# jipolanco/PencilArrays.jl

Hardware: NVIDIA B200
Metric: transpose_GiB_per_s (higher is better)
Workload: dtype c128 (bytes; pure data movement)

## Files before the change

include/pa_b200.h:

```cpp
#ifndef PA_B200_H
#define PA_B200_H

#include <stddef.h>
#include <stdint.h>

#ifdef __cplusplus
extern "C" {
#endif

#define PA_MAX_DIMS 8
#define PA_MAX_TOPO 7
#define PA_UNIQUE_ID_BYTES 128

typedef enum pa_status {
  PA_OK = 0,
  PA_EINVAL = 1,
  PA_EINCOMPAT = 2,
  PA_EDIM = 3,
  PA_ECUDA = 4,
  PA_ENCCL = 5,
  PA_ENOMEM = 6,
  PA_ESTATE = 7,
  PA_ENOGPU = 8
} pa_status;
// ... 79 lines not shown
  int64_t recv_count;
  int64_t remote_recv_offset;
} pa_peer_info;
pa_status pa_plan_get_peer(const pa_plan* plan, int n , pa_peer_info* info);

typedef struct pa_block_desc {
  int nd;
  int64_t extent[PA_MAX_DIMS];
  int64_t src_stride[PA_MAX_DIMS];
  int64_t dst_stride[PA_MAX_DIMS];
  int64_t src_offset;
  int64_t dst_offset;
  int kernel_class;
  int vec_bytes;
} pa_block_desc;
pa_status pa_plan_get_block(const pa_plan* plan, int op, int n ,
                            pa_block_desc* desc);
pa_status pa_plan_get_chunk(const pa_plan* plan, int op, int n, int part, int nparts,
                            pa_block_desc* desc, int64_t* wire_offset, int64_t* wire_bytes);

pa_status pa_pack(pa_plan* plan, int n, const void* src, void* buf, void* stream);
pa_status pa_unpack(pa_plan* plan, int n, const void* recv_buf, void* dst, void* stream);
pa_status pa_copy_self(pa_plan* plan, const void* src, void* dst, void* stream);
pa_status pa_put(pa_plan* plan, int n, const void* src, void* peer_dst, void* stream);
pa_status pa_get(pa_plan* plan, int n, const void* peer_src, void* dst, void* stream);
pa_status pa_put_all(pa_plan* plan, const void* src, void* const* peers, int max_ctas,
                     void* stream);
pa_status pa_get_all(pa_plan* plan, void* const* peers, void* dst, int max_ctas, void* stream);
pa_status pa_permute_local(pa_plan* plan, const void* src, void* dst,
                           void* scratch, void* stream);
pa_status pa_box_copy(int nd, const int64_t* extent, const int64_t* src_stride,
                      const int64_t* dst_stride, int elsize, const void* src,
                      void* dst, void* stream, pa_block_desc* chosen );

pa_status pa_comm_unique_id(void* id128);
pa_status pa_comm_init_rank(const void* id128, int nranks, int rank, pa_comm** out);
pa_status pa_comm_init_local(int nranks, int rank, pa_comm** out);
void pa_comm_destroy(pa_comm* c);
pa_status pa_comm_flags_export(pa_comm* c, void* handle64, int64_t* offset);
pa_status pa_comm_flags_import(pa_comm* c, int rank, const void* handle64, int64_t offset);

#define PA_IPC_HANDLE_BYTES 64
pa_status pa_ipc_export(const void* devptr, void* handle64, int64_t* offset);
pa_status pa_ipc_import(const void* handle64, int64_t offset, void** mapped);
pa_status pa_ipc_release(const void* handle64);
pa_status pa_plan_set_window(pa_plan* plan, const void* local_dst, int n, void* peer_dst);
pa_status pa_plan_set_recv_window(pa_plan* plan, int n, void* peer_recv_buf);

pa_status pa_transpose(pa_plan* plan, pa_comm* comm, const void* src, void* dst,
                       unsigned flags, void* stream);
pa_status pa_wait(pa_plan* plan, void* stream);
pa_status pa_transpose_host(pa_plan* plan, pa_comm* comm, const void* host_src,
                            void* host_dst, unsigned flags);

pa_status pa_host_chain_create(int n, pa_plan* const* plans, pa_comm* comm,
                               pa_host_chain** out);
void pa_host_chain_destroy(pa_host_chain* c);
pa_status pa_host_chain_submit(pa_host_chain* c, const void* host_src, void* host_dst,
                               int64_t* ticket );
pa_status pa_host_chain_wait(pa_host_chain* c, int64_t ticket);
pa_status pa_host_chain_buffer(pa_host_chain* c, int slot, int which, void** devptr,
                               int64_t* bytes);
pa_status pa_host_chain_time_begin(pa_host_chain* c);
pa_status pa_host_chain_time_end(pa_host_chain* c, float* ms);

pa_status pa_io_sizes(const pa_pencil* p, int n_extra, const int64_t* extra_dims, int elsize,
// ... 23 lines not shown
```

pencilarrays.jl_b200/_lib.py:

```python
from __future__ import annotations

import ctypes as C
import os

PA_MAX_DIMS = 8
PA_MAX_TOPO = 7
PA_UNIQUE_ID_BYTES = 128

PA_OK, PA_EINVAL, PA_EINCOMPAT, PA_EDIM, PA_ECUDA, PA_ENCCL, PA_ENOMEM, PA_ESTATE, PA_ENOGPU = range(9)

PA_POINT_TO_POINT = 0
PA_ALLTOALLV = 1
PA_PEER_PUT = 2
PA_PEER_GET = 3
PA_IPC_HANDLE_BYTES = 64

PA_WAITALL = 1
PA_NO_OVERLAP = 2
PA_STAGE_SELF = 4
PA_FFT_FORWARD = 8
PA_FFT_BACKWARD = 16

_HERE = os.path.dirname(os.path.abspath(__file__))
LIB_PATH = os.path.join(_HERE, "libpa_b200.so")


class PlanInfo(C.Structure):
    _fields_ = [
        ("dim", C.c_int), ("nproc", C.c_int), ("self_index", C.c_int), ("same_perm", C.c_int),
        ("elsize", C.c_int), ("method", C.c_int),
        ("length_in", C.c_int64), ("length_out", C.c_int64), ("length_self", C.c_int64),
        ("send_bytes", C.c_int64), ("recv_bytes", C.c_int64),
    ]


class PeerInfo(C.Structure):
    _fields_ = [
        ("world_rank", C.c_int), ("is_self", C.c_int),
        ("send_offset", C.c_int64), ("send_count", C.c_int64),
        ("recv_offset", C.c_int64), ("recv_count", C.c_int64),
        ("remote_recv_offset", C.c_int64),
    ]


class BlockDesc(C.Structure):
    _fields_ = [
        ("nd", C.c_int),
        ("extent", C.c_int64 * PA_MAX_DIMS),
        ("src_stride", C.c_int64 * PA_MAX_DIMS),
        ("dst_stride", C.c_int64 * PA_MAX_DIMS),
        ("src_offset", C.c_int64), ("dst_offset", C.c_int64),
        ("kernel_class", C.c_int), ("vec_bytes", C.c_int),
    ]


class Timings(C.Structure):
    _fields_ = [("total_ms", C.c_float), ("pack_ms", C.c_float),
                ("exchange_ms", C.c_float), ("unpack_ms", C.c_float)]


_P = C.c_void_p
_I64P = C.POINTER(C.c_int64)
_IP = C.POINTER(C.c_int)
SIGNATURES = {
    "pa_version": (C.c_char_p, []),
    "pa_strerror": (C.c_char_p, [C.c_int]),
    "pa_last_error": (C.c_char_p, []),
    "pa_launch_count": (C.c_int64, []),
    "pa_device_count": (C.c_int, []),
    "pa_set_device": (C.c_int, [C.c_int]),
    "pa_set_tunable": (C.c_int, [C.c_char_p, C.c_int64]),
    "pa_dims_create": (C.c_int, [C.c_int, C.c_int, _I64P]),
    "pa_topology_create": (C.c_int, [C.c_int, _I64P, C.c_int, C.POINTER(_P)]),
    "pa_topology_destroy": (None, [_P]),
    "pa_topology_info": (C.c_int, [_P, _IP, _I64P, _IP, _IP, _I64P]),
    "pa_topology_rank_of": (C.c_int, [_P, _I64P, _IP]),
    "pa_topology_line": (C.c_int, [_P, C.c_int, _IP]),
    "pa_pencil_create": (C.c_int, [_P, C.c_int, _I64P, _IP, _IP, _P, C.POINTER(_P)]),
    "pa_pencil_destroy": (None, [_P]),
    "pa_pencil_range": (C.c_int, [_P, _I64P, C.c_int, _I64P, _I64P]),
    "pa_pencil_size_local": (C.c_int, [_P, C.c_int, _I64P]),
    "pa_pencil_buffers": (C.c_int, [_P, C.POINTER(_P), _I64P, C.POINTER(_P), _I64P]),
    "pa_pencil_reserve": (C.c_int, [_P, C.c_int64, C.c_int64]),
    "pa_plan_create": (C.c_int, [_P, _P, C.c_int, _I64P, C.c_int, C.c_int, C.POINTER(_P)]),
    "pa_plan_destroy": (None, [_P]),
    "pa_plan_get_info": (C.c_int, [_P, C.POINTER(PlanInfo)]),
    "pa_plan_get_peer": (C.c_int, [_P, C.c_int, C.POINTER(PeerInfo)]),
    "pa_plan_get_block": (C.c_int, [_P, C.c_int, C.c_int, C.POINTER(BlockDesc)]),
    "pa_plan_get_chunk": (C.c_int, [_P, C.c_int, C.c_int, C.c_int, C.c_int, C.POINTER(BlockDesc),
                                    _I64P, _I64P]),
    "pa_pack": (C.c_int, [_P, C.c_int, _P, _P, _P]),
    "pa_unpack": (C.c_int, [_P, C.c_int, _P, _P, _P]),
    "pa_put": (C.c_int, [_P, C.c_int, _P, _P, _P]),
    "pa_get": (C.c_int, [_P, C.c_int, _P, _P, _P]),
    "pa_put_all": (C.c_int, [_P, _P, C.POINTER(_P), C.c_int, _P]),
    "pa_get_all": (C.c_int, [_P, C.POINTER(_P), _P, C.c_int, _P]),
    "pa_copy_self": (C.c_int, [_P, _P, _P, _P]),
    "pa_permute_local": (C.c_int, [_P, _P, _P, _P, _P]),
    "pa_box_copy": (C.c_int, [C.c_int, _I64P, _I64P, _I64P, C.c_int, _P, _P, _P,
                              C.POINTER(BlockDesc)]),
    "pa_comm_unique_id": (C.c_int, [_P]),
    "pa_comm_init_rank": (C.c_int, [_P, C.c_int, C.c_int, C.POINTER(_P)]),
    "pa_comm_init_local": (C.c_int, [C.c_int, C.c_int, C.POINTER(_P)]),
    "pa_comm_destroy": (None, [_P]),
    "pa_comm_flags_export": (C.c_int, [_P, _P, _I64P]),
    "pa_comm_flags_import": (C.c_int, [_P, C.c_int, _P, C.c_int64]),
    "pa_ipc_export": (C.c_int, [_P, _P, _I64P]),
    "pa_ipc_import": (C.c_int, [_P, C.c_int64, C.POINTER(_P)]),
    "pa_ipc_release": (C.c_int, [_P]),
    "pa_plan_set_window": (C.c_int, [_P, _P, C.c_int, _P]),
    "pa_plan_set_recv_window": (C.c_int, [_P, C.c_int, _P]),
    "pa_transpose": (C.c_int, [_P, _P, _P, _P, C.c_uint, _P]),
    "pa_wait": (C.c_int, [_P, _P]),
    "pa_transpose_host": (C.c_int, [_P, _P, _P, _P, C.c_uint]),
    "pa_host_chain_create": (C.c_int, [C.c_int, C.POINTER(_P), _P, C.POINTER(_P)]),
    "pa_host_chain_destroy": (None, [_P]),
    "pa_host_chain_submit": (C.c_int, [_P, _P, _P, _I64P]),
    "pa_host_chain_wait": (C.c_int, [_P, C.c_int64]),
    "pa_host_chain_time_begin": (C.c_int, [_P]),
    "pa_host_chain_time_end": (C.c_int, [_P, C.POINTER(C.c_float)]),
    "pa_host_chain_buffer": (C.c_int, [_P, C.c_int, C.c_int, C.POINTER(_P), _I64P]),
    "pa_io_sizes": (C.c_int, [_P, C.c_int, _I64P, C.c_int, C.c_int, _I64P, _I64P, _I64P, _I64P, _I64P]),
    "pa_io_run_offset": (C.c_int, [_P, C.c_int, _I64P, C.c_int, C.c_int, C.c_int64, _I64P]),
    "pa_io_write": (C.c_int, [_P, C.c_int, _I64P, C.c_int, C.c_int, _P, C.c_char_p, C.c_int64]),
    "pa_io_read": (C.c_int, [_P, C.c_int, _I64P, C.c_int, C.c_int, _P, C.c_char_p, C.c_int64]),
    "pa_plan_timings": (C.c_int, [_P, C.POINTER(Timings)]),
    "pa_plan_enable_timing": (C.c_int, [_P, C.c_int]),
}


def _load():
    if not os.path.exists(LIB_PATH):
        raise ImportError(
# ... 54 lines not shown
```

pencilarrays.jl_b200/csrc/capi.cpp:

```cpp
#include <algorithm>
#include <new>
#include <vector>

#include "pa_internal.hpp"

using namespace pa;

#define GUARD(expr)                    \
  try {                                \
    expr                               \
  } catch (const std::bad_alloc&) {    \
    set_error("out of host memory");   \
    return PA_ENOMEM;                  \
  } catch (...) {                      \
    set_error("unexpected exception"); \
    return PA_EINVAL;                  \
  }

extern "C" {

const char* pa_version(void) { return "pa_b200 0.2.0 (sm_100a)"; }

const char* pa_strerror(pa_status s) {
  switch (s) {
    case PA_OK: return "success";
    case PA_EINVAL: return "invalid argument";
    case PA_EINCOMPAT: return "pencil configurations are not compatible for transposition";
    case PA_EDIM: return "array dimensions do not match the pencil";
    case PA_ECUDA: return "CUDA error";
    case PA_ENCCL: return "NCCL error";
    case PA_ENOMEM: return "out of memory";
    case PA_ESTATE: return "invalid call sequence";
    case PA_ENOGPU: return "no CUDA device (there is no CPU fallback)";
  }
  return "unknown status";
}

const char* pa_last_error(void) { return last_error(); }
int64_t pa_launch_count(void) { return launch_count(); }
int pa_device_count(void) { return device_count(); }
pa_status pa_set_device(int device) {
  if (device_count() == 0) {
    set_error("no CUDA device");
    return PA_ENOGPU;
  }
  return set_device(device);
}

pa_status pa_set_tunable(const char* name, int64_t value) {
  if (!name) return PA_EINVAL;
  if (!strcmp(name, "remote_ctas")) g_tun.remote_ctas = (int)value;
  else if (!strcmp(name, "box_copy_ctas")) g_tun.box_copy_ctas = (int)value;
  else if (!strcmp(name, "nccl_fences")) g_tun.nccl_fences = (int)value;
  else if (!strcmp(name, "bulk_rows")) g_tun.bulk_rows = (int)value;
  else if (!strcmp(name, "nccl_register")) g_tun.nccl_register = (int)value;
  else if (!strcmp(name, "transpose_tbq")) g_tun.transpose_tbq = (int)value;
  else if (!strcmp(name, "small_block_bytes")) g_tun.small_block_bytes = value;
  else if (!strcmp(name, "transpose_y_fastest")) g_tun.transpose_y_fastest = (int)value;
  else if (!strcmp(name, "multi_put")) g_tun.multi_put = (int)value;
  else if (!strcmp(name, "fft_lines")) g_tun.fft_lines = (int)value;
  else if (!strcmp(name, "oneside_self_ctas")) g_tun.oneside_self_ctas = (int)value;
  else if (!strcmp(name, "p2p_chunks")) g_tun.p2p_chunks = (int)value;
  else if (!strcmp(name, "staged_ctas")) g_tun.staged_ctas = (int)value;
  else if (!strcmp(name, "self_first")) g_tun.self_first = (int)value;
  else if (!strcmp(name, "ipc_exchange")) g_tun.ipc_exchange = (int)value;
  else if (!strcmp(name, "fence_timeout_ms")) g_tun.fence_timeout_ms = value;
  else if (!strcmp(name, "pdl")) g_tun.pdl = (int)value;
  else if (!strcmp(name, "nccl_ctas")) g_tun.nccl_ctas = (int)value;
  else if (!strcmp(name, "host_chunk_bytes")) g_tun.host_chunk_bytes = value;
  else if (!strcmp(name, "host_slots")) g_tun.host_slots = (int)value;
  else {
    set_error("unknown tunable '%s'", name);
    return PA_EINVAL;
  }
  return PA_OK;
}

pa_status pa_dims_create(int nprocs, int M, int64_t* dims) {
  if (nprocs < 1 || M < 1 || M > PA_MAX_TOPO || !dims) {
    set_error("pa_dims_create: bad arguments");
    return PA_EINVAL;
  }
  for (int i = 0; i < M; ++i) dims[i] = 1;
  int64_t primes[64];
  int np = 0;
  int n = nprocs;
  for (int f = 2; (int64_t)f * f <= n; ++f)
    while (n % f == 0) {
      primes[np++] = f;
// ... 406 lines not shown
pa_status pa_permute_local(pa_plan* plan, const void* src, void* dst, void* scratch,
                           void* stream) {
  if (!plan) return PA_EINVAL;
  return permute_local(plan->p, src, dst, scratch, stream);
}

pa_status pa_box_copy(int nd, const int64_t* extent, const int64_t* src_stride,
                      const int64_t* dst_stride, int elsize, const void* src, void* dst,
                      void* stream, pa_block_desc* chosen) {
  if (nd < 0 || nd > PA_MAX_DIMS || (nd > 0 && (!extent || !src_stride || !dst_stride))) {
    set_error("pa_box_copy: 0..%d dimensions", PA_MAX_DIMS);
    return PA_EINVAL;
  }
  if (elsize != 1 && elsize != 2 && elsize != 4 && elsize != 8 && elsize != 16) {
    set_error("pa_box_copy: element size must be 1, 2, 4, 8 or 16");
    return PA_EINVAL;
  }
  BlockCopy b;
  b.elsize = elsize;
  b.nd_raw = nd;
  for (int i = 0; i < nd; ++i) {
    if (extent[i] < 0 || src_stride[i] < 0 || dst_stride[i] < 0) {
      set_error("pa_box_copy: negative extent or stride");
      return PA_EINVAL;
    }
    b.raw[i] = Dim{extent[i], src_stride[i], dst_stride[i]};
  }
  canonicalize(b);
  int vec = 0;
  pa_status s = PA_OK;
  if (src || dst) {
    s = need_gpu();
    if (s != PA_OK) return s;
    s = launch_block(b, src, dst, stream, &vec, g_tun.box_copy_ctas);
  }
  if (chosen) {
    export_block(b, chosen);
    if (vec) chosen->vec_bytes = vec;
  }
  return s;
}

pa_status pa_comm_unique_id(void* id128) {
  if (!id128) return PA_EINVAL;
  return comm_unique_id(id128);
}

pa_status pa_comm_init_rank(const void* id128, int nranks, int rank, pa_comm** out) {
  GUARD({
    if (!id128 || !out || nranks < 1 || rank < 0 || rank >= nranks) return PA_EINVAL;
    Comm* c = nullptr;
    pa_status s = comm_init(id128, nranks, rank, &c);
    if (s != PA_OK) return s;
    *out = new pa_comm{c};
    return PA_OK;
  })
}

pa_status pa_comm_init_local(int nranks, int rank, pa_comm** out) {
  GUARD({
    if (!out || nranks < 1 || rank < 0 || rank >= nranks) return PA_EINVAL;
    Comm* c = nullptr;
    pa_status s = comm_init_local(nranks, rank, &c);
    if (s != PA_OK) return s;
    *out = new pa_comm{c};
    return PA_OK;
  })
}

pa_status pa_comm_flags_export(pa_comm* c, void* handle64, int64_t* offset) {
  if (!c || !handle64 || !offset) return PA_EINVAL;
  return comm_flags_export(c->p, handle64, offset);
}
// ... 171 lines not shown
```

pencilarrays.jl_b200/csrc/kernels.cu:

```cuda
#include <cuda_runtime.h>

#include <atomic>
#include <cstdint>

#include "pa_internal.hpp"

namespace pa {

Tunables g_tun;
static std::atomic<i64> g_launches{0};
i64 launch_count() { return g_launches.load(); }
void count_launch() { g_launches.fetch_add(1); }

constexpr int MAXO = PA_MAX_DIMS - 1;
typedef unsigned long long ull;

struct KParams {
  const char* src;
  char* dst;
  long long ex, ey;
  long long sx_s, sx_d, sy_s, sy_d;
  unsigned tiles_x, tiles_y;
  ull total;
  int no;
  long long oe[MAXO], os[MAXO], od[MAXO];
  int lx_log2, ux_log2;
  int y_fastest;
};

__device__ __forceinline__ void decode_tile(const KParams& p, ull bid, unsigned& tx, unsigned& ty,
                                            const char*& s, char*& d) {
  if (p.y_fastest) {
    ty = (unsigned)(bid % p.tiles_y);
    bid /= p.tiles_y;
    tx = (unsigned)(bid % p.tiles_x);
    bid /= p.tiles_x;
// ... 188 lines not shown
                : make_uint4(r[0].z, r[0].w, r[1].z, r[1].w);
}
__device__ __forceinline__ unsigned comp(const uint4& v, int c) {
  return c == 0 ? v.x : c == 1 ? v.y : c == 2 ? v.z : v.w;
}
template <>
__device__ __forceinline__ uint4 gather_col<4>(const uint4 (&r)[4], int c) {
  return make_uint4(comp(r[0], c), comp(r[1], c), comp(r[2], c), comp(r[3], c));
}
__device__ __forceinline__ uint4 pack_item(const uint32_t (&e)[4]) {
  return make_uint4(e[0], e[1], e[2], e[3]);
}
__device__ __forceinline__ uint4 pack_item(const uint2 (&e)[2]) {
  return make_uint4(e[0].x, e[0].y, e[1].x, e[1].y);
}
__device__ __forceinline__ uint4 pack_item(const uint4 (&e)[1]) { return e[0]; }
__device__ __forceinline__ void unpack_item(const uint4& v, uint32_t (&e)[4]) {
  e[0] = v.x, e[1] = v.y, e[2] = v.z, e[3] = v.w;
}
__device__ __forceinline__ void unpack_item(const uint4& v, uint2 (&e)[2]) {
  e[0] = make_uint2(v.x, v.y), e[1] = make_uint2(v.z, v.w);
}
__device__ __forceinline__ void unpack_item(const uint4& v, uint4 (&e)[1]) { e[0] = v; }

template <int S, int TBQ, bool SE, bool DE>
struct TransBody {
  static constexpr int V = 16 / S;
  static constexpr int TA = 32 * V;
  static constexpr int TB = TBQ * V;
  static constexpr int PITCH = TBQ + 1;
  static constexpr int QI = TBQ / 8;
  static constexpr int SMEM_ITEMS = TA * PITCH;
  static constexpr bool SYNC = true;
  typedef typename Elem<S>::T ET;

  static __device__ __forceinline__ void run(const KParams& p, ull bid, uint4* sm) {
    const int warp = threadIdx.x >> 5, lane = threadIdx.x & 31;
    unsigned tx, ty;
    const char* s;
    char* d;
    decode_tile(p, bid, tx, ty, s, d);
    const long long x0 = (long long)tx * TA, y0 = (long long)ty * TB;

    if constexpr (!SE) {
      const long long xl = x0 + lane * V;
      const bool xok = xl < p.ex;
      uint4 r[QI][V];
#pragma unroll
      for (int qi = 0; qi < QI; ++qi) {
#pragma unroll
        for (int rr = 0; rr < V; ++rr) {
          const long long y = y0 + (long long)(warp + 8 * qi) * V + rr;
          r[qi][rr] = (xok && y < p.ey) ? ld_stream<uint4>(s + y * p.sy_s + xl * S)
                                        : make_uint4(0u, 0u, 0u, 0u);
        }
      }
#pragma unroll
      for (int qi = 0; qi < QI; ++qi) {
        const int q = warp + 8 * qi;
#pragma unroll
        for (int c = 0; c < V; ++c) sm[(c * 32 + lane) * PITCH + q] = gather_col<S>(r[qi], c);
      }
    } else {
      ET r[QI][V][V];
#pragma unroll
      for (int qi = 0; qi < QI; ++qi) {
// ... 10 lines not shown
          }
        }
      }
#pragma unroll
      for (int qi = 0; qi < QI; ++qi) {
        const int q = warp + 8 * qi;
#pragma unroll
        for (int c = 0; c < V; ++c) sm[(c * 32 + lane) * PITCH + q] = pack_item(r[qi][c]);
      }
    }
    __syncthreads();
    if constexpr (!DE) {
      constexpr int IT = TA * TBQ / 256;
#pragma unroll
      for (int k = 0; k < IT; ++k) {
        const int idx = threadIdx.x + 256 * k;
        const int xr = idx / TBQ, qq = idx % TBQ;
        const long long x = SE ? x0 + xr : x0 + (long long)(xr & 31) * V + (xr >> 5);
        const long long y = y0 + (long long)qq * V;
        if (x < p.ex && y < p.ey) st_stream<uint4>(d + x * p.sx_d + y * S, sm[xr * PITCH + qq]);
      }
    } else {
      const ET* sme = reinterpret_cast<const ET*>(sm);
      constexpr int ITE = TA * TB / 256;
#pragma unroll 8
      for (int k = 0; k < ITE; ++k) {
        const int idx = threadIdx.x + 256 * k;
        const int xr = idx / TB, ye = idx % TB;
        const long long x = SE ? x0 + xr : x0 + (long long)(xr & 31) * V + (xr >> 5);
        const long long y = y0 + ye;
        if (x < p.ex && y < p.ey)
          st_stream<ET>(d + x * p.sx_d + y * S, sme[(xr * PITCH + ye / V) * V + (ye % V)]);
      }
    }
  }
};

template <typename ET>
struct ScalarBody {
  static constexpr int SMEM_ITEMS = (32 * 33 * sizeof(ET) + 15) / 16;
  static constexpr bool SYNC = true;
  static __device__ __forceinline__ void run(const KParams& p, ull bid, uint4* smraw) {
    ET(*sm)[33] = reinterpret_cast<ET(*)[33]>(smraw);
    const int a = threadIdx.x & 31, b = threadIdx.x >> 5;
    unsigned tx, ty;
    const char* s;
    char* d;
    decode_tile(p, bid, tx, ty, s, d);
    const long long x0 = (long long)tx * 32, y0 = (long long)ty * 32;
#pragma unroll
    for (int k = 0; k < 4; ++k) {
      const long long x = x0 + a, y = y0 + b + 8 * k;
      if (x < p.ex && y < p.ey)
        sm[b + 8 * k][a] = *reinterpret_cast<const ET*>(s + x * p.sx_s + y * p.sy_s);
    }
    __syncthreads();
#pragma unroll
    for (int k = 0; k < 4; ++k) {
      const long long x = x0 + b + 8 * k, y = y0 + a;
      if (x < p.ex && y < p.ey)
        *reinterpret_cast<ET*>(d + x * p.sx_d + y * p.sy_d) = sm[a][b + 8 * k];
    }
  }
};

template <class B, bool LOOP>
__global__ void __launch_bounds__(256) k_box(const __grid_constant__ KParams p) {
  __shared__ uint4 sm[B::SMEM_ITEMS > 0 ? B::SMEM_ITEMS : 1];
  pdl_enter();
  if constexpr (LOOP) {
    for (ull bid = blockIdx.x; bid < p.total; bid += gridDim.x) {
      B::run(p, bid, sm);
      if (B::SYNC) __syncthreads();
    }
  } else {
    B::run(p, blockIdx.x, sm);
  }
}

__device__ __forceinline__ void flag_signal(ull* remote, ull seq) {
  __threadfence_system();
  asm volatile("red.release.sys.global.max.u64 [%0], %1;" ::"l"(remote), "l"(seq) : "memory");
}
__device__ __forceinline__ void flag_wait(const ull* local, ull seq, ull timeout_ns, int* err) {
  ull t0, now, v;
  asm volatile("mov.u64 %0, %%globaltimer;" : "=l"(t0));
  for (;;) {
    asm volatile("ld.acquire.sys.global.u64 %0, [%1];" : "=l"(v) : "l"(local) : "memory");
    if (v >= seq) return;
    asm volatile("mov.u64 %0, %%globaltimer;" : "=l"(now));
    if (timeout_ns && now - t0 > timeout_ns) {
      if (err) {
        *(volatile int*)err = 1;
        __threadfence_system();
      }
      __trap();
    }
    __nanosleep(100);
  }
}

struct FlagKernelParams {
  int n;
  ull* remote[64];
  ull* local[64];
  ull seq[64];
  int do_signal, do_wait;
  ull timeout_ns;
  int* err;
};
// ... 243 lines not shown
  set_error("kernel launch failed: %s", cudaGetErrorString(e));
  return e == cudaErrorNoDevice || e == cudaErrorInsufficientDriver ? PA_ENOGPU : PA_ECUDA;
}

static pa_status launch_bulk(const BlockCopy& b, KParams& p, cudaStream_t st, int max_ctas) {
  static bool attr_set[64] = {false};
  int dev = 0;
  cudaGetDevice(&dev);
  if (dev < 0 || dev >= 64 || !attr_set[dev]) {
    cudaFuncSetAttribute(k_rows_bulk, cudaFuncAttributeMaxDynamicSharedMemorySize,
                         BULK_STAGES * BULK_CHUNK);
    if (dev >= 0 && dev < 64) attr_set[dev] = true;
  }
  const long long S = b.elsize;
  const long long run = b.d[0].e * S;
  const long long chunk = std::min<long long>(BULK_CHUNK, run);
  p.ex = run;
  p.lx_log2 = (int)chunk;
  p.tiles_x = (unsigned)cdiv(run, chunk);
  p.tiles_y = (unsigned)(b.nd > 1 ? b.d[1].e : 1);
  ull units = (ull)p.tiles_x * p.tiles_y;
  for (int i = 0; i < p.no; ++i) units *= (ull)p.oe[i];
  p.total = units;
  long long ctas = max_ctas > 0 ? max_ctas : (max_ctas < 0 ? -max_ctas : 3) * (long long)sm_count();
  if ((ull)ctas > units) ctas = (long long)units;
  cudaGetLastError();
  k_rows_bulk<<<(unsigned)ctas, 32, BULK_STAGES * BULK_CHUNK, st>>>(p);
  cudaError_t e = cudaGetLastError();
  if (e != cudaSuccess) return launch_err(e);
  count_launch();
  return PA_OK;
}

pa_status launch_block(const BlockCopy& b, const void* src, void* dst, void* stream, int* vec_used,
                       int max_ctas, bool pdl) {
  if (vec_used) *vec_used = 0;
  if (b.klass == KC_EMPTY) return PA_OK;
  KParams p;
  Sel sel;
  pa_status rc = prepare(b, src, dst, p, sel, vec_used);
  if (rc != PA_OK) return rc;
  cudaStream_t st = (cudaStream_t)stream;
  if (p.total == 0) return PA_OK;
  if (sel.fam == F_ROWS && g_tun.bulk_rows && sel.w == 16) {
    if (vec_used) *vec_used = 16;
    return launch_bulk(b, p, st, max_ctas);
  }
  if (max_ctas < 0) max_ctas = -max_ctas * sm_count();
  if (p.total > 0x7fffffffULL && (max_ctas <= 0 || max_ctas > 0x7fffffff))
    max_ctas = 64 * sm_count();
  const bool loop = max_ctas > 0 && p.total > (ull)max_ctas;
  const unsigned grid = loop ? (unsigned)max_ctas : (unsigned)p.total;
  pdl = pdl && g_tun.pdl;
  return dispatch(sel, [&](auto tag) -> pa_status {
    typedef typename decltype(tag)::Body B;
    cudaLaunchConfig_t cfg = {};
    cfg.gridDim = dim3(grid);
    cfg.blockDim = dim3(256);
    cfg.dynamicSmemBytes = 0;
    cfg.stream = st;
    cudaLaunchAttribute at[1];
    at[0].id = cudaLaunchAttributeProgrammaticStreamSerialization;
    at[0].val.programmaticStreamSerializationAllowed = 1;
    cfg.attrs = at;
    cfg.numAttrs = pdl ? 1 : 0;
    cudaError_t e = loop ? cudaLaunchKernelEx(&cfg, k_box<B, true>, p)
                         : cudaLaunchKernelEx(&cfg, k_box<B, false>, p);
    if (e != cudaSuccess) return launch_err(e);
    count_launch();
    return PA_OK;
  });
}

pa_status launch_multi(int nb, const BlockCopy* const* blocks, const void* const* srcs,
                       void* const* dsts, void* stream, int max_ctas, const MultiFlags* mf) {
  if (nb > FLAG_INLINE_MAX) return PA_EINCOMPAT;
  MultiParams mp;
  memset(&mp, 0, sizeof mp);
  Sel sel0;
  bool have = false;
  for (int i = 0; i < nb; ++i) {
    if (blocks[i]->klass == KC_EMPTY) continue;
    KParams p;
    Sel sel;
    pa_status rc = prepare(*blocks[i], srcs[i], dsts[i], p, sel, nullptr);
    if (rc != PA_OK) return rc;
    if (p.total == 0) continue;
    if (p.total > 0x7fffffffULL) return PA_EINCOMPAT;
    if (have && !(sel == sel0)) return PA_EINCOMPAT;
    sel0 = sel;
    have = true;
    mp.kp[mp.nb++] = p;
    mp.max_total = std::max(mp.max_total, p.total);
  }
  if (mf) mp.mf = *mf;
  if (!have) {
    if (!mf || (mf->ready.n == 0 && mf->done.n == 0)) return PA_OK;
    sel0.fam = F_ROWS;
// ... 33 lines not shown
```

pencilarrays.jl_b200/csrc/pa_internal.hpp:

```cpp
#pragma once
#include <cstdint>
#include <cstring>
#include <map>
#include <memory>
#include <string>
#include <vector>

#include "../../include/pa_b200.h"

namespace pa {

using i64 = int64_t;

void set_error(const char* fmt, ...);
const char* last_error();

struct Topology {
  int M = 0;
  i64 dims[PA_MAX_TOPO] = {0};
  int rank = 0;
  int size = 1;
  i64 coords[PA_MAX_TOPO] = {0};

  void coords_of(int r, i64* c) const;
// ... 35 lines not shown
inline void local_data_range(i64 p0, i64 P, i64 N, i64* lo, i64* hi) {
  *lo = (N * p0) / P;
  *hi = (N * (p0 + 1)) / P;
}

struct Dim {
  i64 e;
  i64 ss;
  i64 ds;
};

enum KernelClass { KC_EMPTY = 0, KC_ROWS = 1, KC_TRANSPOSE = 2, KC_TILE_SCALAR = 3 };

struct BlockCopy {
  int nd_raw = 0;
  Dim raw[PA_MAX_DIMS + 1];
  i64 src_off = 0, dst_off = 0;
  int elsize = 0;
  i64 count = 0;

  int nd = 0;
  Dim d[PA_MAX_DIMS + 1];
  int klass = KC_EMPTY;
  int stride_align = 16;
  int src_align = 16;
  int dst_align = 16;
  bool contiguous_both = false;
};

void canonicalize(BlockCopy& b);
BlockCopy sub_block(const BlockCopy& b, int part, int nparts, bool dense_is_dst, i64* dense_off,
                    i64* dense_cnt);

pa_status launch_block(const BlockCopy& b, const void* src, void* dst, void* stream,
                       int* vec_used, int max_ctas = 0, bool pdl = false);

constexpr int FLAG_INLINE_MAX = 8;
struct FlagSet {
  int n;
  unsigned long long* remote[FLAG_INLINE_MAX];
  unsigned long long* local[FLAG_INLINE_MAX];
  unsigned long long seq[FLAG_INLINE_MAX];
};
struct MultiFlags {
  FlagSet ready;
  FlagSet done;
  int wait_done;
  unsigned int* counter;
  unsigned long long timeout_ns;
  int* err;
};
pa_status launch_multi(int nb, const BlockCopy* const* blocks, const void* const* srcs,
                       void* const* dsts, void* stream, int max_ctas, const MultiFlags* mf);

struct Tunables {
  int remote_ctas = -4;
  int box_copy_ctas = 0;
  int transpose_y_fastest = -1;
  int transpose_tbq = 0;
  long long small_block_bytes = 256ll << 20;
  int bulk_rows = 0;
  int nccl_register = 1;
  int nccl_fences = 0;
  int oneside_self_ctas = 0;
  int fft_lines = 0;
  int multi_put = 1;
  int p2p_chunks = 1;
  int self_first = 0;
  int staged_ctas = 0;
  int ipc_exchange = 0;
  long long fence_timeout_ms = 60000;
  int pdl = 1;
  int nccl_ctas = 0;
  long long host_chunk_bytes = 64ll << 20;
  int host_slots = 2;
};
extern Tunables g_tun;

struct Peer {
  int world_rank = -1;
  bool is_self = false;
  i64 send_off = 0, send_cnt = 0;
  i64 recv_off = 0, recv_cnt = 0;
  BlockCopy pack;
  BlockCopy unpack;
  BlockCopy put;
  BlockCopy get;
  i64 remote_recv_off = 0;
};

struct TransposeState;
// ... 88 lines not shown
```

pencilarrays.jl_b200/csrc/plan.cpp:

```cpp
#include <algorithm>
#include <cstdarg>
#include <cstdio>

#include "pa_internal.hpp"

namespace pa {

static thread_local char g_err[512] = {0};
void set_error(const char* fmt, ...) {
  va_list ap;
  va_start(ap, fmt);
  vsnprintf(g_err, sizeof g_err, fmt, ap);
  va_end(ap);
}
const char* last_error() { return g_err; }

void Topology::coords_of(int r, i64* c) const {
  for (int i = M - 1; i >= 0; --i) {
    c[i] = r % dims[i];
    r /= (int)dims[i];
  }
}
int Topology::rank_of(const i64* c) const {
  i64 r = 0;
// ... 60 lines not shown
  } else {
    Dim y = t[j];
    for (int i = j; i > 1; --i) t[i] = t[i - 1];
    t[1] = y;
    b.klass = (t[0].ss == 1 && t[1].ds == 1) ? KC_TRANSPOSE : KC_TILE_SCALAR;
  }
  b.nd = n;
  for (int i = 0; i < n; ++i) b.d[i] = t[i];
  b.contiguous_both = (n == 1 && t[0].ss == 1 && t[0].ds == 1);

  const i64 S = b.elsize;
  int sa = 16, da = 16;
  if (b.klass == KC_ROWS) {
    sa = da = pow2_divisor(t[0].e * S, 16);
    for (int i = 1; i < n; ++i) {
      sa = std::min(sa, pow2_divisor(t[i].ss * S, 16));
      da = std::min(da, pow2_divisor(t[i].ds * S, 16));
    }
  } else if (b.klass == KC_TRANSPOSE) {
    sa = std::min(sa, pow2_divisor(t[0].e * S, 16));
    sa = std::min(sa, pow2_divisor(t[1].ss * S, 16));
    da = std::min(da, pow2_divisor(t[1].e * S, 16));
    da = std::min(da, pow2_divisor(t[0].ds * S, 16));
    for (int i = 2; i < n; ++i) {
      sa = std::min(sa, pow2_divisor(t[i].ss * S, 16));
      da = std::min(da, pow2_divisor(t[i].ds * S, 16));
    }
  } else {
    sa = da = (int)std::min<i64>(S, 16);
  }
  b.src_align = sa;
  b.dst_align = da;
  b.stride_align = std::min(sa, da);
}

BlockCopy sub_block(const BlockCopy& b, int part, int nparts, bool dense_is_dst, i64* dense_off,
                    i64* dense_cnt) {
  BlockCopy c = b;
  int j = -1;
  for (int i = b.nd_raw - 1; i >= 0; --i)
    if (b.raw[i].e > 1) {
      j = i;
      break;
    }
  if (b.count == 0 || j < 0) {
    if (part != 0) {
      for (int i = 0; i < c.nd_raw; ++i) c.raw[i].e = (i == 0) ? 0 : c.raw[i].e;
      if (c.nd_raw == 0) {
        c.nd_raw = 1;
        c.raw[0] = Dim{0, 1, 1};
      }
    }
    canonicalize(c);
    if (dense_off) *dense_off = 0;
    if (dense_cnt) *dense_cnt = c.count;
    return c;
  }
  const i64 e = b.raw[j].e;
  const i64 c0 = e * part / nparts, c1 = e * (part + 1) / nparts;
  c.raw[j].e = c1 - c0;
  c.src_off += c0 * b.raw[j].ss;
  c.dst_off += c0 * b.raw[j].ds;
  canonicalize(c);
  const i64 dense_stride = dense_is_dst ? b.raw[j].ds : b.raw[j].ss;
  if (dense_off) *dense_off = c0 * dense_stride;
  if (dense_cnt) *dense_cnt = (c1 - c0) * dense_stride;
// ... 244 lines not shown
```

Before: 3091.

## Add persistent pipelined transpose kernel and optional copy-engine box copies

Adds a persistent transpose kernel that launches one wave of resident CTAs. Each CTA prefetches the next tile into registers while it writes the current tile out of shared memory, which is meant to hide global load latency and remove per-tile launch and tail costs. It is enabled by default for 16-byte element transposes when no CTA cap is given. It also adds an optional copy-engine path that issues box copies as cudaMemcpy2D/3D calls, with a host helper and microbenchmarks. The pipelined kernel trades lower occupancy from the register prefetch for the overlap.

```diff
diff --git a/include/pa_b200.h b/include/pa_b200.h
--- a/include/pa_b200.h
+++ b/include/pa_b200.h
@@ -135,6 +135,14 @@
 pa_status pa_box_copy(int nd, const int64_t* extent, const int64_t* src_stride,
                       const int64_t* dst_stride, int elsize, const void* src,
                       void* dst, void* stream, pa_block_desc* chosen );
+typedef struct pa_copy_op {
+  int64_t src_offset, dst_offset;
+  int64_t width, height, depth;
+  int64_t src_pitch, src_height;
+  int64_t dst_pitch, dst_height;
+} pa_copy_op;
+pa_status pa_copy_engine_ops(const pa_block_desc* box, int elsize, pa_copy_op* ops, int cap,
+                             int* n);
 
 pa_status pa_comm_unique_id(void* id128);
 pa_status pa_comm_init_rank(const void* id128, int nranks, int rank, pa_comm** out);
diff --git a/pencilarrays.jl_b200/_lib.py b/pencilarrays.jl_b200/_lib.py
--- a/pencilarrays.jl_b200/_lib.py
+++ b/pencilarrays.jl_b200/_lib.py
@@ -54,6 +54,11 @@
     ]
 
 
+class CopyOp(C.Structure):
+    _fields_ = [(f, C.c_int64) for f in ("src_offset", "dst_offset", "width", "height", "depth",
+                                         "src_pitch", "src_height", "dst_pitch", "dst_height")]
+
+
 class Timings(C.Structure):
     _fields_ = [("total_ms", C.c_float), ("pack_ms", C.c_float),
                 ("exchange_ms", C.c_float), ("unpack_ms", C.c_float)]
@@ -99,6 +104,7 @@
     "pa_permute_local": (C.c_int, [_P, _P, _P, _P, _P]),
     "pa_box_copy": (C.c_int, [C.c_int, _I64P, _I64P, _I64P, C.c_int, _P, _P, _P,
                               C.POINTER(BlockDesc)]),
+    "pa_copy_engine_ops": (C.c_int, [C.POINTER(BlockDesc), C.c_int, C.POINTER(CopyOp), C.c_int, _IP]),
     "pa_comm_unique_id": (C.c_int, [_P]),
     "pa_comm_init_rank": (C.c_int, [_P, C.c_int, C.c_int, C.POINTER(_P)]),
     "pa_comm_init_local": (C.c_int, [C.c_int, C.c_int, C.POINTER(_P)]),
diff --git a/pencilarrays.jl_b200/csrc/capi.cpp b/pencilarrays.jl_b200/csrc/capi.cpp
--- a/pencilarrays.jl_b200/csrc/capi.cpp
+++ b/pencilarrays.jl_b200/csrc/capi.cpp
@@ -51,10 +51,12 @@
   if (!name) return PA_EINVAL;
   if (!strcmp(name, "remote_ctas")) g_tun.remote_ctas = (int)value;
   else if (!strcmp(name, "box_copy_ctas")) g_tun.box_copy_ctas = (int)value;
+  else if (!strcmp(name, "box_copy_engine")) g_tun.box_copy_engine = (int)value;
   else if (!strcmp(name, "nccl_fences")) g_tun.nccl_fences = (int)value;
   else if (!strcmp(name, "bulk_rows")) g_tun.bulk_rows = (int)value;
   else if (!strcmp(name, "nccl_register")) g_tun.nccl_register = (int)value;
   else if (!strcmp(name, "transpose_tbq")) g_tun.transpose_tbq = (int)value;
+  else if (!strcmp(name, "transpose_pipe")) g_tun.transpose_pipe = (int)value;
   else if (!strcmp(name, "small_block_bytes")) g_tun.small_block_bytes = value;
   else if (!strcmp(name, "transpose_y_fastest")) g_tun.transpose_y_fastest = (int)value;
   else if (!strcmp(name, "multi_put")) g_tun.multi_put = (int)value;
@@ -527,13 +529,61 @@
   if (src || dst) {
     s = need_gpu();
     if (s != PA_OK) return s;
-    s = launch_block(b, src, dst, stream, &vec, g_tun.box_copy_ctas);
+    s = g_tun.box_copy_engine ? launch_engine(b, src, dst, stream)
+                              : launch_block(b, src, dst, stream, &vec, g_tun.box_copy_ctas);
   }
   if (chosen) {
     export_block(b, chosen);
     if (vec) chosen->vec_bytes = vec;
   }
   return s;
+}
+
+pa_status pa_copy_engine_ops(const pa_block_desc* box, int elsize, pa_copy_op* ops, int cap,
+                             int* n) {
+  if (!box || !n || cap < 0 || (cap > 0 && !ops) || box->nd < 0 || box->nd > PA_MAX_DIMS) {
+    set_error("pa_copy_engine_ops: bad arguments");
+    return PA_EINVAL;
+  }
+  if (elsize != 1 && elsize != 2 && elsize != 4 && elsize != 8 && elsize != 16) {
+    set_error("pa_copy_engine_ops: element size must be 1, 2, 4, 8 or 16");
+    return PA_EINVAL;
+  }
+  BlockCopy b;
+  b.elsize = elsize;
+  b.nd_raw = box->nd;
+  for (int i = 0; i < box->nd; ++i) {
+    if (box->extent[i] < 0 || box->src_stride[i] < 0 || box->dst_stride[i] < 0) {
+      set_error("pa_copy_engine_ops: negative extent or stride");
+      return PA_EINVAL;
+    }
+    b.raw[i] = Dim{box->extent[i], box->src_stride[i], box->dst_stride[i]};
+  }
+  b.src_off = box->src_offset;
+  b.dst_off = box->dst_offset;
+  canonicalize(b);
+  std::vector<PitchedCopy> v;
+  try {
+    if (!pitched_copies(b, v)) return PA_EINVAL;
+  } catch (const std::bad_alloc&) {
+    set_error("out of host memory");
+    return PA_ENOMEM;
+  }
+  *n = (int)v.size();
+  for (int i = 0; i < std::min(cap, *n); ++i) {
+    const PitchedCopy& o = v[i];
+    pa_copy_op& r = ops[i];
+    r.src_offset = o.src_off;
+    r.dst_offset = o.dst_off;
+    r.width = o.width;
+    r.height = o.height;
+    r.depth = o.depth;
+    r.src_pitch = o.src_pitch;
+    r.src_height = o.src_height;
+    r.dst_pitch = o.dst_pitch;
+    r.dst_height = o.dst_height;
+  }
+  return PA_OK;
 }
 
 pa_status pa_comm_unique_id(void* id128) {
diff --git a/pencilarrays.jl_b200/csrc/kernels.cu b/pencilarrays.jl_b200/csrc/kernels.cu
--- a/pencilarrays.jl_b200/csrc/kernels.cu
+++ b/pencilarrays.jl_b200/csrc/kernels.cu
@@ -2,6 +2,7 @@
 
 #include <atomic>
 #include <cstdint>
+#include <type_traits>
 
 #include "pa_internal.hpp"
 
@@ -256,6 +257,7 @@
   static constexpr int QI = TBQ / 8;
   static constexpr int SMEM_ITEMS = TA * PITCH;
   static constexpr bool SYNC = true;
+  static constexpr int PIPE_CTAS = QI * V <= 2 ? 8 : QI * V <= 4 ? 4 : 3;
   typedef typename Elem<S>::T ET;
 
   static __device__ __forceinline__ void run(const KParams& p, ull bid, uint4* sm) {
@@ -332,6 +334,64 @@
         if (x < p.ex && y < p.ey)
           st_stream<ET>(d + x * p.sx_d + y * S, sme[(xr * PITCH + ye / V) * V + (ye % V)]);
       }
+    }
+  }
+
+  static __device__ __forceinline__ void load_tile(const KParams& p, ull bid, uint4 (&r)[QI][V],
+                                                   char*& d, long long& x0, long long& y0) {
+    const int warp = threadIdx.x >> 5, lane = threadIdx.x & 31;
+    unsigned tx, ty;
+    const char* s;
+    decode_tile(p, bid, tx, ty, s, d);
+    x0 = (long long)tx * TA;
+    y0 = (long long)ty * TB;
+    const long long xl = x0 + lane * V;
+    const bool xok = xl < p.ex;
+#pragma unroll
+    for (int qi = 0; qi < QI; ++qi) {
+#pragma unroll
+      for (int rr = 0; rr < V; ++rr) {
+        const long long y = y0 + (long long)(warp + 8 * qi) * V + rr;
+        r[qi][rr] = (xok && y < p.ey) ? ld_stream<uint4>(s + y * p.sy_s + xl * S)
+                                      : make_uint4(0u, 0u, 0u, 0u);
+      }
+    }
+  }
+  static __device__ __forceinline__ void run_pipelined(const KParams& p, uint4* sm) {
+    static_assert(!SE && !DE, "pipelined tiles move 16-byte items on both sides");
+    const int warp = threadIdx.x >> 5, lane = threadIdx.x & 31;
+    ull bid = blockIdx.x;
+    uint4 r[QI][V];
+    char* d;
+    long long x0, y0;
+    load_tile(p, bid, r, d, x0, y0);
+    for (;;) {
+#pragma unroll
+      for (int qi = 0; qi < QI; ++qi) {
+        const int q = warp + 8 * qi;
+#pragma unroll
+        for (int c = 0; c < V; ++c) sm[(c * 32 + lane) * PITCH + q] = gather_col<S>(r[qi], c);
+      }
+      __syncthreads();
+      const ull next = bid + gridDim.x;
+      char* dn = nullptr;
+      long long xn = 0, yn = 0;
+      if (next < p.total) load_tile(p, next, r, dn, xn, yn);
+      constexpr int IT = TA * TBQ / 256;
+#pragma unroll
+      for (int k = 0; k < IT; ++k) {
+        const int idx = threadIdx.x + 256 * k;
+        const int xr = idx / TBQ, qq = idx % TBQ;
+        const long long x = x0 + (long long)(xr & 31) * V + (xr >> 5);
+        const long long y = y0 + (long long)qq * V;
+        if (x < p.ex && y < p.ey) st_stream<uint4>(d + x * p.sx_d + y * S, sm[xr * PITCH + qq]);
+      }
+      if (next >= p.total) break;
+      __syncthreads();
+      bid = next;
+      d = dn;
+      x0 = xn;
+      y0 = yn;
     }
   }
 };
@@ -376,6 +436,13 @@
   } else {
     B::run(p, blockIdx.x, sm);
   }
+}
+
+template <class B>
+__global__ void __launch_bounds__(256, B::PIPE_CTAS) k_trans_pipe(const __grid_constant__ KParams p) {
+  __shared__ uint4 sm[B::SMEM_ITEMS];
+  pdl_enter();
+  B::run_pipelined(p, sm);
 }
 
 __device__ __forceinline__ void flag_signal(ull* remote, ull seq) {
@@ -685,6 +752,39 @@
   return PA_OK;
 }
 
+pa_status launch_engine(const BlockCopy& b, const void* src, void* dst, void* stream) {
+  std::vector<PitchedCopy> ops;
+  if (!pitched_copies(b, ops)) return PA_EINVAL;
+  cudaStream_t st = (cudaStream_t)stream;
+  for (const PitchedCopy& o : ops) {
+    char* s = (char*)src + o.src_off;
+    char* d = (char*)dst + o.dst_off;
+    cudaError_t e;
+    if (o.height == 1 && o.depth == 1) {
+      e = cudaMemcpyAsync(d, s, o.width, cudaMemcpyDefault, st);
+    } else if (o.depth == 1) {
+      e = cudaMemcpy2DAsync(d, o.dst_pitch, s, o.src_pitch, o.width, o.height, cudaMemcpyDefault, st);
+    } else {
+      cudaMemcpy3DParms p = {};
+      p.srcPtr = make_cudaPitchedPtr(s, o.src_pitch, o.width, o.src_height);
+      p.dstPtr = make_cudaPitchedPtr(d, o.dst_pitch, o.width, o.dst_height);
+      p.extent = make_cudaExtent(o.width, o.height, o.depth);
+      p.kind = cudaMemcpyDefault;
+      e = cudaMemcpy3DAsync(&p, st);
+    }
+    if (e != cudaSuccess) {
+      set_error("copy engine: %s", cudaGetErrorString(e));
+      return e == cudaErrorNoDevice || e == cudaErrorInsufficientDriver ? PA_ENOGPU : PA_ECUDA;
+    }
+  }
+  return PA_OK;
+}
+
+template <class B>
+struct Pipelined : std::false_type {};
+template <int S, int TBQ>
+struct Pipelined<TransBody<S, TBQ, false, false>> : std::true_type {};
+
 pa_status launch_block(const BlockCopy& b, const void* src, void* dst, void* stream, int* vec_used,
                        int max_ctas, bool pdl) {
   if (vec_used) *vec_used = 0;
@@ -704,6 +804,7 @@
     max_ctas = 64 * sm_count();
   const bool loop = max_ctas > 0 && p.total > (ull)max_ctas;
   const unsigned grid = loop ? (unsigned)max_ctas : (unsigned)p.total;
+  const bool alone = pdl;
   pdl = pdl && g_tun.pdl;
   return dispatch(sel, [&](auto tag) -> pa_status {
     typedef typename decltype(tag)::Body B;
@@ -717,6 +818,22 @@
     at[0].val.programmaticStreamSerializationAllowed = 1;
     cfg.attrs = at;
     cfg.numAttrs = pdl ? 1 : 0;
+    if constexpr (Pipelined<B>::value) {
+      if (alone && max_ctas == 0 && g_tun.transpose_pipe) {
+        static int per_sm = 0;
+        if (per_sm == 0 &&
+            (cudaOccupancyMaxActiveBlocksPerMultiprocessor(&per_sm, k_trans_pipe<B>, 256, 0) !=
+                 cudaSuccess ||
+             per_sm < 1))
+          per_sm = 1;
+        const ull resident = (ull)per_sm * (ull)sm_count();
+        cfg.gridDim = dim3((unsigned)std::min<ull>(p.total, resident));
+        cudaError_t e = cudaLaunchKernelEx(&cfg, k_trans_pipe<B>, p);
+        if (e != cudaSuccess) return launch_err(e);
+        count_launch();
+        return PA_OK;
+      }
+    }
     cudaError_t e = loop ? cudaLaunchKernelEx(&cfg, k_box<B, true>, p)
                          : cudaLaunchKernelEx(&cfg, k_box<B, false>, p);
     if (e != cudaSuccess) return launch_err(e);
diff --git a/pencilarrays.jl_b200/csrc/pa_internal.hpp b/pencilarrays.jl_b200/csrc/pa_internal.hpp
--- a/pencilarrays.jl_b200/csrc/pa_internal.hpp
+++ b/pencilarrays.jl_b200/csrc/pa_internal.hpp
@@ -91,6 +91,15 @@
 BlockCopy sub_block(const BlockCopy& b, int part, int nparts, bool dense_is_dst, i64* dense_off,
                     i64* dense_cnt);
 
+struct PitchedCopy {
+  i64 src_off, dst_off;
+  i64 width, height, depth;
+  i64 src_pitch, src_height;
+  i64 dst_pitch, dst_height;
+};
+bool pitched_copies(const BlockCopy& b, std::vector<PitchedCopy>& out);
+pa_status launch_engine(const BlockCopy& b, const void* src, void* dst, void* stream);
+
 pa_status launch_block(const BlockCopy& b, const void* src, void* dst, void* stream,
                        int* vec_used, int max_ctas = 0, bool pdl = false);
 
@@ -115,7 +124,9 @@
 struct Tunables {
   int remote_ctas = -4;
   int box_copy_ctas = 0;
+  int box_copy_engine = 0;
   int transpose_y_fastest = -1;
+  int transpose_pipe = 1;
   int transpose_tbq = 0;
   long long small_block_bytes = 256ll << 20;
   int bulk_rows = 0;
diff --git a/pencilarrays.jl_b200/csrc/plan.cpp b/pencilarrays.jl_b200/csrc/plan.cpp
--- a/pencilarrays.jl_b200/csrc/plan.cpp
+++ b/pencilarrays.jl_b200/csrc/plan.cpp
@@ -116,6 +116,55 @@
   b.src_align = sa;
   b.dst_align = da;
   b.stride_align = std::min(sa, da);
+}
+
+bool pitched_copies(const BlockCopy& b, std::vector<PitchedCopy>& out) {
+  out.clear();
+  if (b.klass == KC_EMPTY) return true;
+  const int y0 = b.klass == KC_ROWS ? 1 : 0;
+  const i64 S = b.elsize;
+  PitchedCopy c{};
+  c.width = y0 ? b.d[0].e * S : S;
+  c.height = c.depth = 1;
+  c.src_pitch = c.dst_pitch = c.width;
+  c.src_height = c.dst_height = 1;
+  int outer = y0;
+  if (b.nd > y0) {
+    const Dim& y = b.d[y0];
+    c.height = y.e;
+    c.src_pitch = y.ss * S;
+    c.dst_pitch = y.ds * S;
+    if (c.src_pitch < c.width || c.dst_pitch < c.width) {
+      set_error("copy engine: runs of %lld bytes overlap (pitch %lld / %lld bytes)", (long long)c.width,
+                (long long)c.src_pitch, (long long)c.dst_pitch);
+      return false;
+    }
+    c.src_height = c.dst_height = y.e;
+    outer = y0 + 1;
+    if (b.nd > y0 + 1) {
+      const Dim& z = b.d[y0 + 1];
+      if (z.ss % y.ss == 0 && z.ds % y.ds == 0 && z.ss / y.ss >= y.e && z.ds / y.ds >= y.e) {
+        c.depth = z.e;
+        c.src_height = z.ss / y.ss;
+        c.dst_height = z.ds / y.ds;
+        outer = y0 + 2;
+      }
+    }
+  }
+  i64 k[PA_MAX_DIMS + 1] = {0};
+  for (;;) {
+    PitchedCopy o = c;
+    o.src_off = b.src_off * S;
+    o.dst_off = b.dst_off * S;
+    for (int i = outer; i < b.nd; ++i) {
+      o.src_off += k[i] * b.d[i].ss * S;
+      o.dst_off += k[i] * b.d[i].ds * S;
+    }
+    out.push_back(o);
+    int i = outer;
+    while (i < b.nd && ++k[i] == b.d[i].e) k[i++] = 0;
+    if (i >= b.nd) return true;
+  }
 }
 
 BlockCopy sub_block(const BlockCopy& b, int part, int nparts, bool dense_is_dst, i64* dense_off,
diff --git a/profiles/ce_microbench.py b/profiles/ce_microbench.py
--- /dev/null
+++ b/profiles/ce_microbench.py
@@ -0,0 +1,213 @@
+#!/usr/bin/env python
+import ctypes as C
+import os
+import subprocess
+import sys
+
+import torch
+
+ROOT = os.path.dirname(os.path.dirname(os.path.abspath(__file__)))
+sys.path.insert(0, ROOT)
+import pencilarrays_b200 as pa
+from pencilarrays_b200._lib import lib, check, i64arr
+
+GIB = 1 << 30
+SHAPES = [("8 KiB runs of 16 KiB rows (cfg4 N=2 x->y pack)", 16, 512, 1024, 256, 512),
+          ("4 KiB runs of 16 KiB rows (cfg4 N=8 x->y pack)", 16, 256, 1024, 256, 1024),
+          ("2 KiB runs of 8 KiB rows (cfg5 N=8 x->y pack)", 4, 512, 2048, 512, 1024)]
+
+
+def set_engine(on):
+    check(lib.pa_set_tunable(b"box_copy_engine", 1 if on else 0))
+
+
+def box(ext, ss, ds, es, src, dst, stream, engine):
+    set_engine(engine)
+    check(lib.pa_set_device(stream.device.index))
+    check(lib.pa_box_copy(len(ext), i64arr(ext), i64arr(ss), i64arr(ds), es, C.c_void_p(src),
+                          C.c_void_p(dst), C.c_void_p(stream.cuda_stream), None))
+
+
+def contiguous(nbytes):
+    return [nbytes // 16], [1], [1], 16
+
+
+def pitched(shape, nslices=None):
+    _, es, run, row, h, d = shape
+    d = nslices or d
+    return [run, h, d], [1, row, row * h], [1, run, run * h], es
+
+
+def timeit(fns, streams, reps=10):
+    for f in fns:
+        f()
+    for s in streams:
+        s.synchronize()
+    ev = []
+    for s in streams:
+        a, b = torch.cuda.Event(enable_timing=True), torch.cuda.Event(enable_timing=True)
+        a.record(s)
+        ev.append((a, b, s))
+    for a, _, s in ev:
+        for a2, _, s2 in ev:
+            if s2.device == s.device and s2 is not s:
+                s2.wait_event(a)
+    for _ in range(reps):
+        for f in fns:
+            f()
+    for a, b, s in ev:
+        b.record(s)
+    for s in streams:
+        s.synchronize()
+    per_dev = {}
+    for a, b, s in ev:
+        per_dev.setdefault(s.device.index, []).append((a, b))
+    spans = []
+    for pairs in per_dev.values():
+        a0 = pairs[0][0]
+        spans.append(max(a0.elapsed_time(b) for _, b in pairs))
+    return max(spans) / reps
+
+
+ROWS = []
+
+
+def rec(name, ms, nbytes, note=""):
+    gbs = nbytes / ms / 1e6
+    ROWS.append((name, ms, gbs))
+    print(f"{name:78s} {ms:8.3f} ms {gbs:8.1f} GB/s {note}", flush=True)
+
+
+def skip(name, why):
+    print(f"{name:78s} not measured ({why})", flush=True)
+
+
+def card():
+    try:
+        q = subprocess.run(["nvidia-smi", "--query-gpu=index,name,power.limit,clocks.max.sm",
+                            "--format=csv,noheader"], capture_output=True, text=True, timeout=30)
+        return q.stdout.strip()
+    except Exception as e:
+        return f"nvidia-smi unavailable: {e}"
+
+
+def main():
+    ng = torch.cuda.device_count()
+    assert ng >= 1, "needs a CUDA device"
+    print("cards:", card().replace("\n", " | "))
+    print(f"devices visible: {ng}; torch {torch.__version__}")
+    devs = list(range(min(ng, 4)))
+    src = {d: torch.empty(4 * GIB, dtype=torch.uint8, device=f"cuda:{d}") for d in devs}
+    dst = {d: torch.empty(GIB, dtype=torch.uint8, device=f"cuda:{d}") for d in devs}
+    for d in devs:
+        src[d].random_()
+    if ng >= 2:
+        for d in devs:
+            for e in devs:
+                if d != e:
+                    dst[e][:16].copy_(src[d][:16])
+        for d in devs:
+            torch.cuda.synchronize(d)
+    st = {d: torch.cuda.Stream(device=d) for d in devs}
+    st2 = {d: torch.cuda.Stream(device=d) for d in devs}
+    S = lambda d: src[d].data_ptr()
+    D = lambda d: dst[d].data_ptr()
+
+    kinds = [("contiguous 1 GiB", contiguous(GIB))] + [(s[0], pitched(s)) for s in SHAPES]
+    for label, (ext, ss, ds, es) in kinds:
+        for eng, tag in ((True, "CE"), (False, "SM")):
+            ms = timeit([lambda: box(ext, ss, ds, es, S(0), D(0), st[0], eng)], [st[0]])
+            rec(f"{tag} local 0->0, {label}", ms, GIB)
+            if ng < 2:
+                skip(f"{tag} 0->1 / both directions, {label}", "needs 2 GPUs")
+                continue
+            ms = timeit([lambda: box(ext, ss, ds, es, S(0), D(1), st[0], eng)], [st[0]])
+            rec(f"{tag} 0->1, {label}", ms, GIB)
+            ms = timeit([lambda: box(ext, ss, ds, es, S(0), D(1), st[0], eng),
+                         lambda: box(ext, ss, ds, es, S(1), D(0), st[1], eng)], [st[0], st[1]])
+            rec(f"{tag} both directions (per direction), {label}", ms, GIB)
+
+    shp = SHAPES[1]
+    third = max(1, GIB // 3 // (shp[2] * shp[1] * shp[4]))
+    ext, ss, ds, es = pitched(shp, third)
+    nb3 = ext[0] * ext[1] * ext[2] * es
+    if ng >= 4:
+        peer_st = {p: torch.cuda.Stream(device=0) for p in (1, 2, 3)}
+        for eng, tag in ((True, "CE"), (False, "SM")):
+            ms = timeit([lambda p=p: box(ext, ss, ds, es, S(0), D(p), peer_st[p], eng) for p in (1, 2, 3)],
+                        list(peer_st.values()))
+            rec(f"{tag} 0->{{1,2,3}} one stream per peer, 4 KiB runs", ms, 3 * nb3)
+        chunks = 8
+        ce = pitched(shp, third // chunks)
+
+        def interleaved():
+            for c in range(chunks):
+                for p in (1, 2, 3):
+                    off = c * ce[0][0] * ce[0][1] * ce[0][2] * es
+                    box(ce[0], ce[1], ce[2], es, S(0) + off * 4, D(p) + off, st[0], True)
+        ms = timeit([interleaved], [st[0]])
+        rec(f"CE 0->{{1,2,3}} {chunks} chunks per peer interleaved on one stream", ms,
+            3 * chunks * ce[0][0] * ce[0][1] * ce[0][2] * es)
+    else:
+        skip("CE / SM 0->{1,2,3}: one stream per peer vs interleaved on one stream", "needs 4 GPUs")
+
+    text, tss, tds = [256, 256, 2048], [1, 256, 65536], [256, 1, 65536]
+    k3 = lambda: box(text, tss, tds, 16, S(0), S(0) + 2 * GIB, st2[0], False)
+    ms_k3 = timeit([k3], [st2[0]])
+    rec("SM K3 transpose (2,1,3) 2 GiB alone (bytes read + written)", ms_k3, 4 * GIB)
+    tgt = 1 if ng >= 2 else 0
+    aux = torch.empty(GIB, dtype=torch.uint8, device="cuda:0").random_()
+    ext, ss, ds, es = pitched(SHAPES[1], 256)
+    ce = lambda: box(ext, ss, ds, es, aux.data_ptr(), D(tgt), st[0], True)
+    nce = ext[0] * ext[1] * ext[2] * es
+    ms_ce = timeit([ce], [st[0]])
+    rec(f"CE 0->{tgt} 256 MiB 4 KiB runs alone", ms_ce, nce)
+    ms_both = timeit([k3, ce], [st2[0], st[0]])
+    rec(f"K3 || CE 0->{tgt}: wall (K3 bytes + CE bytes)", ms_both, 4 * GIB + nce,
+        f"(alone, one after the other: {ms_k3 + ms_ce:.3f} ms)")
+
+    flag = torch.zeros(64, dtype=torch.int64, device="cuda:0")
+    cu = C.CDLL("libcuda.so.1")
+    cu.cuStreamWriteValue64.argtypes = [C.c_void_p, C.c_uint64, C.c_uint64, C.c_uint]
+    seq = [0]
+
+    def write_value(s):
+        seq[0] += 1
+        with torch.cuda.device(s.device):
+            r = cu.cuStreamWriteValue64(C.c_void_p(s.cuda_stream), C.c_uint64(flag.data_ptr()),
+                                        C.c_uint64(seq[0]), 0)
+        if r != 0:
+            raise RuntimeError(f"cuStreamWriteValue64 returned CUresult {r}")
+
+    def kernel_flag(s):
+        with torch.cuda.stream(s):
+            flag[:1].fill_(seq[0])
+
+    for mib in (16, 64, 256):
+        n = GIB // (mib << 20)
+        chunk = mib << 20
+        for sig, sname in ((None, "no signal"), (write_value, "cuStreamWriteValue64"),
+                           (kernel_flag, "one-word kernel")):
+            def run():
+                for i in range(n):
+                    box([chunk // 16], [1], [1], 16, S(0) + i * chunk, D(tgt) + i * chunk, st[0], True)
+                    if sig:
+                        sig(st[0])
+            label = f"CE 0->{tgt} 1 GiB in {n} x {mib} MiB, {sname} after each"
+            try:
+                rec(label, timeit([run], [st[0]]), GIB)
+            except RuntimeError as e:
+                skip(label, str(e))
+
+    half = GIB // 2
+    ce_h = lambda: box([half // 16], [1], [1], 16, S(0), D(tgt), st[0], True)
+    sm_h = lambda: box([half // 16], [1], [1], 16, S(0) + half, D(tgt) + half, st2[0], False)
+    rec(f"CE 0->{tgt} 512 MiB alone", timeit([ce_h], [st[0]]), half)
+    rec(f"SM 0->{tgt} 512 MiB alone", timeit([sm_h], [st2[0]]), half)
+    rec(f"CE || SM 0->{tgt}, 512 MiB each (sum of both)", timeit([ce_h, sm_h], [st[0], st2[0]]), GIB)
+    set_engine(False)
+    print("cards:", card().replace("\n", " | "))
+
+
+if __name__ == "__main__":
+    main()
diff --git a/profiles/prof_pipe.py b/profiles/prof_pipe.py
--- /dev/null
+++ b/profiles/prof_pipe.py
@@ -0,0 +1,95 @@
+#!/usr/bin/env python
+import os
+import subprocess
+import sys
+
+import torch
+
+ROOT = os.path.dirname(os.path.dirname(os.path.abspath(__file__)))
+sys.path.insert(0, ROOT)
+import pencilarrays_b200 as pa
+
+LEGS = ["x->y", "y->z", "z->y", "y->x"]
+
+
+def card():
+    q = subprocess.run(["nvidia-smi", "--query-gpu=name,power.limit,clocks.max.sm", "--format=csv,noheader"],
+                       capture_output=True, text=True)
+    return q.stdout.strip()
+
+
+def main():
+    torch.cuda.set_device(0)
+    print("card:", card())
+    topo = pa.MPITopology(pa.COMM_SELF, (1, 1))
+    px = pa.Pencil(topo, (512, 512, 512), (2, 3))
+    py = pa.Pencil(px, decomp_dims=(1, 3), permute=pa.Permutation(2, 1, 3))
+    pz = pa.Pencil(py, decomp_dims=(1, 2), permute=pa.Permutation(3, 2, 1))
+    ux, uy, uz = (pa.PencilArray.undef(torch.complex128, p) for p in (px, py, pz))
+    ux.data.view(torch.float64).normal_(generator=torch.Generator(device="cuda").manual_seed(42))
+    orig = ux.data.clone()
+    ts = [pa.Transposition(d, s) for d, s in ((uy, ux), (uz, uy), (uy, uz), (ux, uy))]
+    nb = 2 * ux.data.numel() * 16
+
+    def steps(k):
+        ev = [[torch.cuda.Event(enable_timing=True) for _ in range(5)] for _ in range(k)]
+        for e in ev:
+            e[0].record()
+            for i, t in enumerate(ts):
+                pa.transpose_(t)
+                e[i + 1].record()
+        torch.cuda.synchronize()
+        return [sum(e[i].elapsed_time(e[i + 1]) for e in ev) / k for i in range(4)]
+
+    res = {0: [], 1: []}
+    outs = {}
+    for rnd in range(6):
+        for mode in (0, 1) if rnd % 2 == 0 else (1, 0):
+            pa.set_tunable("transpose_pipe", mode)
+            steps(3)
+            res[mode].append(steps(20))
+            pa.transpose_(ts[0])
+            pa.transpose_(ts[1])
+            torch.cuda.synchronize()
+            outs[mode] = (uy.data.clone(), uz.data.clone())
+            pa.transpose_(ts[2])
+            pa.transpose_(ts[3])
+            torch.cuda.synchronize()
+            assert torch.equal(ux.data.view(torch.uint8), orig.view(torch.uint8)), "round trip"
+    same = all(torch.equal(a.view(torch.uint8), b.view(torch.uint8)) for a, b in zip(outs[0], outs[1]))
+    print(f"uy, uz identical between transpose_pipe 0 and 1: {same}")
+    for mode, label in ((0, "one tile per CTA (transpose_pipe=0)"), (1, "pipelined wave (transpose_pipe=1)")):
+        rows = res[mode]
+        step = [sum(r) for r in rows]
+        legs = [sum(r[i] for r in rows) / len(rows) for i in range(4)]
+        print(f"{label}: ms/step per round " + " ".join(f"{s:.4f}" for s in step) +
+              f"; mean {sum(step) / len(step):.4f} ms = {4 * nb / 2 / 2**30 / (sum(step) / len(step) * 1e-3):.1f} GiB/s")
+        print("   legs " + "  ".join(f"{n} {m:.4f} ms ({nb / m / 1e6:.0f} GB/s)" for n, m in zip(LEGS, legs)))
+    q1 = pa.Pencil(topo, (256, 256, 256), (2, 3))
+    srcs = [pa.PencilArray.undef(torch.float64, q1) for _ in range(6)]
+    for a in srcs:
+        a.data.normal_()
+    for perm in ((2, 1, 3), (2, 3, 1), (3, 2, 1), (3, 1, 2), (1, 3, 2)):
+        q2 = pa.Pencil(q1, decomp_dims=(1, 3), permute=pa.Permutation(*perm))
+        dsts = [pa.PencilArray.undef(torch.float64, q2) for _ in range(6)]
+        tl = [pa.Transposition(d, s) for d, s in zip(dsts, srcs)]
+        line = []
+        for mode in (0, 1, 0, 1):
+            pa.set_tunable("transpose_pipe", mode)
+            for t in tl:
+                pa.transpose_(t)
+            a, b = torch.cuda.Event(enable_timing=True), torch.cuda.Event(enable_timing=True)
+            a.record()
+            for _ in range(4):
+                for t in tl:
+                    pa.transpose_(t)
+            b.record()
+            torch.cuda.synchronize()
+            line.append(f"{mode}: {a.elapsed_time(b) / 24:.4f}")
+        print(f"256^3 f64 perm {perm} ms/launch  " + "  ".join(line))
+    pa.set_tunable("transpose_pipe", 1)
+    print("card:", card())
+
+
+if __name__ == "__main__":
+    main()
```

Result: slower. 2711 (median of 6 runs) (-12.3%).
